# sergiventosa/ts-PWS

Measured on AMD Instinct MI355X. Metric: stacked samples/s (Morlet ts-PWS, 10k×131072) + % HBM roofline, 1/2/4/8 GPU, higher is better.
Workload: dtype f64; 1 GPU; 10000 traces/GPU x 131072 samples, Morlet w0=pi*sqrt(2/ln2) V=4 J=14, two-stage K=10 + unbiased phase coherence (BASELINE configs[2]); HBM-resident float32 traces; traces_total=10000, traces_per_gpu=10000, parallelism=one GPU: no collective, world_size=1

## Files before the change

### include/tspws_hip.h

```cpp
#ifndef TSPWS_HIP_H
#define TSPWS_HIP_H

#include <stddef.h>
#include <stdint.h>
#include "ts_pws1f_lib.h"

#ifdef __cplusplus
extern "C" {
#endif

enum {
	TSPWS_OK        = 0,
	TSPWS_E_ARG     = -1,
	TSPWS_E_NOMEM   = 4,
	TSPWS_E_NODEV   = 5,
	TSPWS_E_HIP     = 6,
	TSPWS_E_FRAME   = 7
};

typedef struct tspws_hip_plan tspws_hip_plan;

typedef struct {
	int      type;
	unsigned S, V, J, N;
	double   s0, b0, w0;
	double   Cpsi;
	size_t   ncoef;
	size_t   ntaps;
	int      device;
} tspws_hip_frame_info;

int         tspws_hip_device_count(void);
const char *tspws_hip_last_error(void);
int  tspws_hip_alloc(void **d_ptr, size_t bytes, int device);
int  tspws_hip_free(void *d_ptr);
int  tspws_hip_upload(void *d_dst, const void *h_src, size_t bytes, void *stream);
int  tspws_hip_download(void *h_dst, const void *d_src, size_t bytes, void *stream);
int  tspws_hip_zero(void *d_ptr, size_t bytes, void *stream);
int  tspws_hip_sync(void *stream);


void tspws_resolve_params(t_tsPWS *p, unsigned nsamp, float dt);

int  tspws_hip_plan_create(tspws_hip_plan **plan, int type, unsigned J, unsigned V, unsigned N,
                           double s0, double b0, double w0, int uni, int device);
void tspws_hip_plan_destroy(tspws_hip_plan *plan);
int  tspws_hip_plan_info(const tspws_hip_plan *plan, tspws_hip_frame_info *info);
int  tspws_hip_plan_tables(const tspws_hip_plan *plan, double *scale, unsigned *L, int *c, int *cd,
                           unsigned *D, unsigned *Ns);
int  tspws_hip_plan_taps(const tspws_hip_plan *plan, double *h_w, double *h_wd);

int  tspws_hip_fold(float *d_sigall, size_t mtr, size_t max, size_t ld, void *stream);
int  tspws_hip_remove_mean(float *d_sigall, size_t mtr, size_t max, size_t ld, void *stream);

int  tspws_hip_partial_stacks(tspws_hip_plan *plan, const float *d_sigall, size_t ld,
                              size_t mtr_local, size_t first, size_t mtr_global, unsigned Kmax,
                              double *d_P, size_t ldP, void *stream);

int  tspws_hip_partial_stacks_range(tspws_hip_plan *plan, const float *d_sigall, size_t ld,
                                    size_t mtr_local, size_t first, size_t mtr_global, unsigned Kmax,
                                    unsigned g_begin, unsigned g_end, double *d_P, size_t ldP, void *stream);

int  tspws_hip_forward_f64(tspws_hip_plan *plan, const double *d_x, size_t ntr, size_t ld, double *d_Y, void *stream);
int  tspws_hip_forward_f32(tspws_hip_plan *plan, const float  *d_x, size_t ntr, size_t ld, double *d_Y, void *stream);
unsigned tspws_hip_spectral_first_scale(const tspws_hip_plan *plan, unsigned nsmax);
unsigned tspws_hip_spectral_end_scale(const tspws_hip_plan *plan);
unsigned tspws_hip_spectral_transform_length(const tspws_hip_plan *plan);
unsigned tspws_hip_spectral_choice(const tspws_hip_plan *plan, size_t ntr);
int  tspws_hip_forward_spectral_f64(tspws_hip_plan *plan, const double *d_x, size_t ntr, size_t ld, double *d_Y, unsigned nsmax, void *stream);
int  tspws_hip_forward_spectral_f32(tspws_hip_plan *plan, const float  *d_x, size_t ntr, size_t ld, double *d_Y, unsigned nsmax, void *stream);
int  tspws_hip_inverse(tspws_hip_plan *plan, const double *d_Y, size_t nrec, double *d_x, void *stream);
typedef struct {
	unsigned items;
	unsigned per_scale;
	unsigned waves;
	unsigned waves_lds;
	unsigned waves_fast;
	unsigned generic;
} tspws_hip_inverse_info_t;
int  tspws_hip_inverse_info(const tspws_hip_plan *plan, tspws_hip_inverse_info_t *info);

int  tspws_hip_accumulate(tspws_hip_plan *plan, const double *d_Y, size_t ntr, double *d_ST, double *d_PS,
                          int zero_first, void *stream);
int  tspws_hip_stacks_double(tspws_hip_plan *plan, const double *d_P, unsigned K, size_t ldP,
                             double *d_ST, double *d_PS, void *stream);
int  tspws_hip_stacks_float(tspws_hip_plan *plan, const float *d_sigall, size_t mtr, size_t ld,
                            double *d_ST, double *d_PS, void *stream);
int  tspws_hip_weight(tspws_hip_plan *plan, double *d_OUT, const double *d_ST, const double *d_PS,
                      unsigned K, unsigned M, double wu, int unbiased, void *stream);
int  tspws_hip_epilogue(float *d_ls, float *d_tsPWS, const double *d_x_st, const double *d_x_out,
                        size_t N, unsigned mtr, void *stream);

int  tspws_hip_stack_local(tspws_hip_plan *plan, const t_tsPWS *p, const float *d_sigall, size_t ld,
                           size_t mtr_local, size_t first, size_t mtr_global, void *stream);
int  tspws_hip_reduce_buffer(tspws_hip_plan *plan, const t_tsPWS *p, size_t mtr_global,
                             double **d_buf, size_t *ndoubles);
int  tspws_hip_stack_finish(tspws_hip_plan *plan, const t_tsPWS *p, size_t mtr_global,
                            float *d_ls, float *d_tsPWS, void *stream);

int  tspws_hip_stack_finish_range(tspws_hip_plan *plan, const t_tsPWS *p, size_t mtr_global,
                                  unsigned g_begin, unsigned g_end, void *stream);
int  tspws_hip_stack_finish_tail(tspws_hip_plan *plan, const t_tsPWS *p, size_t mtr_global,
                                 float *d_ls, float *d_tsPWS, void *stream);

int  tspws_hip_stack(tspws_hip_plan *plan, const t_tsPWS *p, const float *d_sigall, size_t ld, size_t mtr,
                     float *d_ls, float *d_tsPWS, void *stream);
int  tspws_hip_stack_batch(tspws_hip_plan *plan, const t_tsPWS *p, const float *d_sigall, size_t ld, const size_t *h_first, unsigned B,
                           float *d_ls, float *d_tsPWS, void *stream);
typedef struct {
	unsigned single_pass;
	unsigned two_stage_pass;
	unsigned looped;
	unsigned empty;
	unsigned rounds;
// ... 187 lines not shown
```

### ts-pws_amd/__init__.py

```python
import ctypes as C
import os
import subprocess

_HERE = os.path.dirname(os.path.abspath(__file__))
ROOT = os.path.dirname(_HERE)
LIB_PATH = os.environ.get("TSPWS_LIB_PATH") or os.path.join(_HERE, "lib", "libtspws_hip.so")

time_t = C.c_long


class t_tsPWS(C.Structure):
    _fields_ = [
        ("type", C.c_int), ("uni", C.c_uint), ("J", C.c_uint), ("V", C.c_uint),
        ("s0", C.c_double), ("b0", C.c_double), ("w0", C.c_double), ("wu", C.c_double),
        ("fmin", C.c_double), ("Q", C.c_double), ("cycle", C.c_double),
        ("w0set", C.c_int), ("lrm", C.c_int), ("bin", C.c_int), ("lkinst", C.c_int),
        ("lVfix", C.c_int), ("ls0fix", C.c_int), ("lb0fix", C.c_int), ("verbose", C.c_int),
        ("fold", C.c_int), ("unbiased", C.c_int), ("convergence", C.c_int),
        ("subsmpl_N", C.c_uint), ("subsmpl_p", C.c_double),
        ("jackknife_n", C.c_uint), ("jackknife_d", C.c_uint), ("obin", C.c_uint),
        ("AllSteps", C.c_int), ("Nmax", C.c_uint), ("Kmax", C.c_uint),
        ("kinst", C.c_char_p), ("filein", C.c_char_p), ("fileout", C.c_char_p), ("fileconv", C.c_char_p),
    ]


class FrameInfo(C.Structure):
    _fields_ = [
        ("type", C.c_int), ("S", C.c_uint), ("V", C.c_uint), ("J", C.c_uint), ("N", C.c_uint),
        ("s0", C.c_double), ("b0", C.c_double), ("w0", C.c_double), ("Cpsi", C.c_double),
        ("ncoef", C.c_size_t), ("ntaps", C.c_size_t), ("device", C.c_int),
    ]


class InverseInfo(C.Structure):
    _fields_ = [("items", C.c_uint), ("per_scale", C.c_uint), ("waves", C.c_uint), ("waves_lds", C.c_uint), ("waves_fast", C.c_uint),
                ("generic", C.c_uint)]


class TspwsError(RuntimeError):
    pass


def build(verbose=False):
    out = subprocess.run(["make", "-C", _HERE, "all"], capture_output=True, text=True)
    if verbose or out.returncode:
        print(out.stdout + out.stderr)
    if out.returncode:
        raise TspwsError("building libtspws_hip.so failed")
    return LIB_PATH


_lib = None

_vp, _u, _d, _sz, _i, _f = C.c_void_p, C.c_uint, C.c_double, C.c_size_t, C.c_int, C.c_float
SYMBOLS = {
    "tspws_main": (_i, [_vp, _vp, _vp]),
    "tspws_hip_device_count": (_i, []),
    "tspws_hip_last_error": (C.c_char_p, []),
    "tspws_hip_alloc": (_i, [C.POINTER(_vp), _sz, _i]),
    "tspws_hip_free": (_i, [_vp]),
    "tspws_hip_upload": (_i, [_vp, _vp, _sz, _vp]),
    "tspws_hip_download": (_i, [_vp, _vp, _sz, _vp]),
    "tspws_hip_zero": (_i, [_vp, _sz, _vp]),
    "tspws_hip_sync": (_i, [_vp]),
    "tspws_resolve_params": (None, [_vp, _u, _f]),
    "tspws_hip_plan_create": (_i, [C.POINTER(_vp), _i, _u, _u, _u, _d, _d, _d, _i, _i]),
    "tspws_hip_plan_destroy": (None, [_vp]),
    "tspws_hip_plan_info": (_i, [_vp, _vp]),
    "tspws_hip_plan_tables": (_i, [_vp] + [_vp] * 6),
    "tspws_hip_plan_taps": (_i, [_vp, _vp, _vp]),
    "tspws_hip_fold": (_i, [_vp, _sz, _sz, _sz, _vp]),
    "tspws_hip_remove_mean": (_i, [_vp, _sz, _sz, _sz, _vp]),
    "tspws_hip_partial_stacks": (_i, [_vp, _vp, _sz, _sz, _sz, _sz, _u, _vp, _sz, _vp]),
    "tspws_hip_partial_stacks_range": (_i, [_vp, _vp, _sz, _sz, _sz, _sz, _u, _u, _u, _vp, _sz, _vp]),
    "tspws_hip_forward_f64": (_i, [_vp, _vp, _sz, _sz, _vp, _vp]),
    "tspws_hip_forward_f32": (_i, [_vp, _vp, _sz, _sz, _vp, _vp]),
    "tspws_hip_spectral_first_scale": (_u, [_vp, _u]),
    "tspws_hip_spectral_end_scale": (_u, [_vp]),
    "tspws_hip_spectral_transform_length": (_u, [_vp]),
    "tspws_hip_spectral_choice": (_u, [_vp, _sz]),
    "tspws_hip_forward_spectral_f64": (_i, [_vp, _vp, _sz, _sz, _vp, _u, _vp]),
    "tspws_hip_forward_spectral_f32": (_i, [_vp, _vp, _sz, _sz, _vp, _u, _vp]),
    "tspws_hip_inverse": (_i, [_vp, _vp, _sz, _vp, _vp]),
    "tspws_hip_inverse_info": (_i, [_vp, _vp]),
    "tspws_hip_accumulate": (_i, [_vp, _vp, _sz, _vp, _vp, _i, _vp]),
    "tspws_hip_stacks_double": (_i, [_vp, _vp, _u, _sz, _vp, _vp, _vp]),
    "tspws_hip_stacks_float": (_i, [_vp, _vp, _sz, _sz, _vp, _vp, _vp]),
    "tspws_hip_weight": (_i, [_vp, _vp, _vp, _vp, _u, _u, _d, _i, _vp]),
    "tspws_hip_epilogue": (_i, [_vp, _vp, _vp, _vp, _sz, _u, _vp]),
    "tspws_hip_stack_local": (_i, [_vp, _vp, _vp, _sz, _sz, _sz, _sz, _vp]),
    "tspws_hip_reduce_buffer": (_i, [_vp, _vp, _sz, C.POINTER(_vp), C.POINTER(_sz)]),
    "tspws_hip_stack_finish": (_i, [_vp, _vp, _sz, _vp, _vp, _vp]),
    "tspws_hip_stack_finish_range": (_i, [_vp, _vp, _sz, _u, _u, _vp]),
    "tspws_hip_stack_finish_tail": (_i, [_vp, _vp, _sz, _vp, _vp, _vp]),
    "tspws_hip_stack": (_i, [_vp, _vp, _vp, _sz, _sz, _vp, _vp, _vp]),
    "tspws_hip_stack_batch": (_i, [_vp, _vp, _vp, _sz, _vp, _u, _vp, _vp, _vp]),
    "tspws_hip_stack_batch_stats": (_i, [_vp, _vp]),
    "tspws_hip_profile_begin": (_i, [_vp, _sz]),
    "tspws_hip_profile_read": (_i, [_vp, _vp, _vp, _sz, C.POINTER(_sz)]),
    "tspws_hip_profile_end": (_i, [_vp, C.POINTER(_d), C.POINTER(_sz)]),
    "tspws_hip_stream_launches": (_i, [_vp]),
    "tspws_jackknife_plan": (_i, [_vp, _vp, _sz, _u, _u, _u]),
    "tspws_hip_jackknife": (_i, [_vp, _vp, _vp, _sz, _sz, _vp, _u, _vp, _vp, _vp, _vp]),
    "tspws_hip_stack_jackknife": (_i, [_vp, _vp, _vp, _sz, _sz, _vp, _vp, _vp, _u, _vp, _vp, _vp, _vp]),
    "tspws_main_release": (None, []),
    "tspws_main_on": (_i, [_i, _vp, _vp, _vp]),
    "tspws_main_cached_devices": (C.c_ulonglong, []),
    "tspws_hip_finish_shard": (_i, [_vp, _vp, _sz, _u, _u, C.POINTER(_u), C.POINTER(_u)]),
    "tspws_hip_stack_finish_scales": (_i, [_vp, _vp, _sz, _u, _u, _vp, _vp]),
    "tspws_hip_jackknife_buffer": (_i, [_vp, _vp, _u, C.POINTER(_vp), C.POINTER(_sz)]),
    "tspws_hip_jackknife_local": (_i, [_vp, _vp, _vp, _sz, _sz, _sz, _sz, _vp, _u, _vp]),
    "tspws_hip_jackknife_finish": (_i, [_vp, _vp, _sz, _vp, _u, _u, _u, _vp, _vp, _vp, _vp]),
    "tspws_selection_classes": (_i, [_vp, _u, _sz, _vp, _vp, C.POINTER(_u)]),
    "tspws_hip_jackknife_single": (_i, [_vp, _vp, _vp, _sz, _sz, _vp, _u, _vp, _vp, _vp, _vp]),
    "tspws_hip_jackknife_batch": (_i, [_vp, _vp, _vp, _sz, _vp, _u, _vp, _u, _vp, _vp, _vp, _vp, _vp, _vp]),
    "tspws_hip_jackknife_batch_stats": (_i, [_vp, _vp]),
    "tspws_hip_jackknife_batch_two_stage": (_i, [_vp, _vp, _vp, _sz, _vp, _u, _vp, _u, _vp, _vp, _vp, _vp, _vp, _vp]),
    "tspws_hip_jackknife_batch_two_stage_stats": (_i, [_vp, _vp]),
    "tspws_subsampling_plan": (_i, [_vp, _sz, _sz]),
    "tspws_hip_subsample": (_i, [_vp, _vp, _vp, _sz, _sz, _u, _vp, _vp, _vp]),
    "tspws_hip_subsample_sel": (_i, [_vp, _vp, _vp, _sz, _sz, _u, _vp, _vp, _vp, _vp]),
    "tspws_subsampling_plan_batch": (_i, [_vp, _vp, _u, _u, _d]),
    "tspws_hip_subsample_batch_sel": (_i, [_vp, _vp, _vp, _sz, _vp, _u, _u, _vp, _vp, _vp, _vp, _vp]),
    "tspws_hip_subsample_batch": (_i, [_vp, _vp, _vp, _sz, _vp, _u, _u, _vp, _vp, _vp, _vp]),
    "tspws_hip_subsample_batch_stats": (_i, [_vp, _vp]),
    "tspws_bootstrap_plan": (_i, [_vp, _sz]),
    "tspws_bootstrap_plan_batch": (_i, [_vp, _vp, _u, _u]),
    "tspws_hip_bootstrap_batch_cnt": (_i, [_vp, _vp, _vp, _sz, _vp, _u, _u, _vp, _vp, _vp, _vp, _vp, _vp]),
    "tspws_hip_bootstrap_batch": (_i, [_vp, _vp, _vp, _sz, _vp, _u, _u, _vp, _vp, _vp, _vp, _vp]),
    "tspws_hip_bootstrap_batch_stats": (_i, [_vp, _vp]),
    "tspws_hip_weighted_stack_batch": (_i, [_vp, _vp, _vp, _sz, _vp, _u, _u, _vp, _vp, _vp, _vp, _vp, _vp]),
    "tspws_hip_weighted_stack_batch_stats": (_i, [_vp, _vp]),
    "tspws_weights_from_scores": (_i, [_vp, _vp, _vp, _u, _i, _d]),
    "tspws_hip_replica_bands": (_i, [_vp, _vp, _sz, _u, _u, _vp, _vp, _u, _vp, _vp]),
    "tspws_hip_replica_bands_stats": (_i, [_vp, _vp]),
    "tspws_hip_trace_scores": (_i, [_vp, _vp, _sz, _vp, _u, _vp, _sz, _u, _sz, _sz, _vp, _vp, _vp]),
    "tspws_hip_trace_scores_stats": (_i, [_vp, _vp]),
    "tspws_selection_from_scores": (_i, [_vp, _vp, _vp, _vp, _u, _i, _d]),
    "tspws_hip_selective_stack_batch": (_i, [_vp, _vp, _vp, _sz, _vp, _u, _i, _i, _d, _u, _sz, _sz, _vp, _vp, _vp, _vp, _vp, _vp]),
    "tspws_hip_convergence": (_i, [_vp, _vp, _vp, _sz, _sz, _vp, _vp, _vp, _vp, _vp, _vp, _vp, _vp, _vp]),
    "tspws_hip_convergence_batch": (_i, [_vp, _vp, _vp, _sz, _vp, _u, _vp, _vp, _vp, _vp, _vp, _vp, _vp, _vp, _vp]),
    "tspws_hip_convergence_batch_stats": (_i, [_vp, _vp]),
    "tspws_hip_synth": (_i, [_vp, _sz, _sz, _sz, C.c_uint64, _sz, _vp]),
    "tspws_hip_comm_create": (_i, [C.POINTER(_vp), _i, _vp]),
    "tspws_hip_comm_destroy": (None, [_vp]),
    "tspws_hip_comm_size": (_i, [_vp]),
    "tspws_hip_comm_device": (_i, [_vp, _i]),
    "tspws_hip_comm_stream": (_vp, [_vp, _i]),
    "tspws_hip_comm_backend": (C.c_char_p, [_vp]),
    "tspws_hip_allreduce_f64": (_i, [_vp, _vp, _sz, _vp]),
    "tspws_hip_reduce_f64": (_i, [_vp, _vp, _sz, _i, _vp]),
    "tspws_shard_range": (None, [_sz, _u, _u, C.POINTER(_sz), C.POINTER(_sz)]),
    "tspws_hip_multi_create": (_i, [C.POINTER(_vp), _i, _vp, _i, _u, _u, _u, _d, _d, _d, _i]),
    "tspws_hip_multi_destroy": (None, [_vp]),
    "tspws_hip_multi_comm": (_vp, [_vp]),
    "tspws_hip_multi_plan": (_vp, [_vp, _i]),
    "tspws_hip_multi_upload": (_i, [_vp, _vp, _sz, _sz, C.POINTER(_vp), C.POINTER(_vp), C.POINTER(_vp)]),
    "tspws_hip_multi_prologue": (_i, [_vp, _vp, _sz, _sz, _sz, _i, _i]),
    "tspws_hip_multi_stack": (_i, [_vp, _vp, _vp, _sz, _sz, _vp, _vp]),
    "tspws_hip_multi_stack_jackknife": (_i, [_vp, _vp, _vp, _sz, _sz, _vp, _vp, _vp, _u, _vp, _vp, _vp]),
}


def load():
    global _lib
    if _lib is None:
        if not os.path.exists(LIB_PATH):
            raise TspwsError(f"{LIB_PATH} is missing: run __graft_entry__.build() / make -C ts-pws_amd")
        try:
            import torch
        except ImportError:
            pass
        lib = C.CDLL(LIB_PATH)
        for name, (res, args) in SYMBOLS.items():
            fn = getattr(lib, name)
            fn.restype, fn.argtypes = res, args
        _lib = lib
    return _lib


def check(rc, what=""):
    if rc:
        raise TspwsError(f"{what} failed with code {rc}: {load().tspws_hip_last_error().decode()}")


def resolve(params, nsamp, dt=1.0):
    p = t_tsPWS.from_buffer_copy(params)
    load().tspws_resolve_params(C.byref(p), nsamp, dt)
    return p


def shard_range(mtr_global, rank, world):
    first = rank * mtr_global // world
    last = (rank + 1) * mtr_global // world
    return first, last - first


class Plan:

    def __init__(self, params, N, device=0):
        self.lib = load()
        self.params = t_tsPWS.from_buffer_copy(params)
        h = C.c_void_p()
        p = self.params
        check(self.lib.tspws_hip_plan_create(C.byref(h), p.type, p.J, p.V, N, p.s0, p.b0, p.w0, int(p.uni), device), "plan_create")
        self.h = h
        info = FrameInfo()
        check(self.lib.tspws_hip_plan_info(self.h, C.byref(info)), "plan_info")
        self.info = info
        self.N, self.S, self.ncoef, self.ntaps, self.Cpsi = N, info.S, info.ncoef, info.ntaps, info.Cpsi
        self.device = device

    def tables(self):
        import numpy as np
        S = self.S
        t = dict(scale=np.zeros(S), L=np.zeros(S, np.uint32), c=np.zeros(S, np.int32), cd=np.zeros(S, np.int32),
# ... 41 lines not shown
        return t.data_ptr()

    def stacks(self, traces):
        import numpy as np
        import torch
        if traces.dtype not in (torch.float32, torch.float64):
            raise TspwsError(f"traces must be float32 or float64 [mtr][{self.N}], got {traces.dtype}")
        mtr, ld = self._traces(traces, traces.dtype)
        if not mtr:
            raise TspwsError("stacks needs at least one row")
        fn = self.lib.tspws_hip_stacks_float if traces.dtype == torch.float32 else self.lib.tspws_hip_stacks_double
        ST = torch.full((2 * self.ncoef,), float("nan"), dtype=torch.float64, device=traces.device)
        PS = torch.full((2 * self.ncoef,), float("nan"), dtype=torch.float64, device=traces.device)
        check(fn(self.h, traces.data_ptr(), mtr, ld, ST.data_ptr(), PS.data_ptr(), self._stream()), "stacks")
        torch.cuda.synchronize(traces.device)
        return ST.cpu().numpy().view(np.complex128), PS.cpu().numpy().view(np.complex128)

    def inverse_info(self):
        info = InverseInfo()
        check(self.lib.tspws_hip_inverse_info(self.h, C.byref(info)), "inverse_info")
        return {k: int(getattr(info, k)) for k, _ in InverseInfo._fields_}

    def inverse(self, Y):
        import numpy as np
        import torch
        if isinstance(Y, np.ndarray):
            if Y.dtype != np.complex128 or Y.ndim != 2 or Y.shape[1] != self.ncoef or not Y.shape[0]:
                raise TspwsError(f"Y must be complex128 [nrec >= 1][{self.ncoef}], got {Y.dtype} {Y.shape}")
            Yd = torch.as_tensor(np.ascontiguousarray(Y), device=f"cuda:{self.device}")
        elif isinstance(Y, torch.Tensor):
            if Y.dtype != torch.complex128 or Y.dim() != 2 or Y.shape[1] != self.ncoef or not Y.shape[0]:
                raise TspwsError(f"Y must be complex128 [nrec >= 1][{self.ncoef}], got {Y.dtype} {tuple(Y.shape)}")
            if not Y.is_cuda or (Y.device.index or 0) != self.device or not Y.is_contiguous():
                raise TspwsError(f"Y must be a contiguous tensor on cuda:{self.device}, got {Y.device}")
            Yd = Y
        else:
            raise TspwsError("Y must be a complex128 numpy array or device tensor")
        x = torch.full((Yd.shape[0], self.N), float("nan"), dtype=torch.float64, device=Yd.device)
        check(self.lib.tspws_hip_inverse(self.h, Yd.data_ptr(), Yd.shape[0], x.data_ptr(), self._stream()), "inverse")
        torch.cuda.synchronize(Yd.device)
        return x.cpu().numpy() if isinstance(Y, np.ndarray) else x

    def stack_local(self, traces, first=0, mtr_global=None):
        mtr, ld = self._traces(traces)
        mtr_global = mtr if mtr_global is None else mtr_global
        check(self.lib.tspws_hip_stack_local(self.h, C.byref(self.params), traces.data_ptr(), ld, mtr, first, mtr_global, self._stream()),
              "stack_local")

    def partial_stacks_range(self, traces, first, mtr_global, g_begin, g_end):
        mtr, ld = self._traces(traces)
        buf = self.reduce_buffer(mtr_global)
        check(self.lib.tspws_hip_partial_stacks_range(self.h, traces.data_ptr(), ld, mtr, first, mtr_global, self.params.Kmax, g_begin, g_end,
                                                      buf.data_ptr(), self.N, self._stream()), "partial_stacks_range")

    def stack_finish(self, mtr_global, ls, ts):
        check(self.lib.tspws_hip_stack_finish(self.h, C.byref(self.params), mtr_global, self._out(ls, "ls"), self._out(ts, "ts"), self._stream()),
              "stack_finish")

    def stack_finish_range(self, mtr_global, g_begin, g_end):
        check(self.lib.tspws_hip_stack_finish_range(self.h, C.byref(self.params), mtr_global, g_begin, g_end, self._stream()),
              "stack_finish_range")

    def stack_finish_tail(self, mtr_global, ls, ts):
        check(self.lib.tspws_hip_stack_finish_tail(self.h, C.byref(self.params), mtr_global, self._out(ls, "ls"), self._out(ts, "ts"),
                                                   self._stream()), "stack_finish_tail")

    @staticmethod
    def _sel(sel, C_, mtr_global):
        import numpy as np
        sel = np.ascontiguousarray(sel, dtype=np.int8)
        if sel.shape != (C_, mtr_global):
            raise TspwsError(f"selection must be [{C_}][{mtr_global}] (replica x trace of the WHOLE ensemble), got {sel.shape}")
        return sel

    def jackknife_buffer(self, C_):
        import torch
        ptr, n = C.c_void_p(), C.c_size_t()
        check(self.lib.tspws_hip_jackknife_buffer(self.h, C.byref(self.params), C_, C.byref(ptr), C.byref(n)), "jackknife_buffer")
        return _as_tensor(ptr.value, n.value, torch.float64, self.device)

    def jackknife_local(self, traces, first, mtr_global, sel):
        mtr, ld = self._traces(traces)
        sel = self._sel(sel, sel.shape[0], mtr_global)
        check(self.lib.tspws_hip_jackknife_local(self.h, C.byref(self.params), traces.data_ptr(), ld, mtr, first, mtr_global, sel.ctypes.data,
                                                 sel.shape[0], self._stream()), "jackknife_local")

    def jackknife_finish(self, mtr_global, sel, c_begin, c_end, ls_out, ts_out, mtr_out):
        import torch
        import numpy as np
        sel = self._sel(sel, sel.shape[0], mtr_global)
        if not isinstance(mtr_out, np.ndarray) or mtr_out.dtype != np.uint32 or mtr_out.shape != (sel.shape[0],) or not mtr_out.flags.c_contiguous:
            raise TspwsError(f"mtr_out must be a contiguous uint32 numpy array of {sel.shape[0]} entries")
        for t, name in ((ls_out, "ls_out"), (ts_out, "ts_out")):
            if t.dtype != torch.float32 or tuple(t.shape) != (sel.shape[0], self.N) or not t.is_contiguous() or not t.is_cuda or \
                    (t.device.index or 0) != self.device:
                raise TspwsError(f"{name} must be a contiguous float32 [{sel.shape[0]}][{self.N}] tensor on cuda:{self.device}")
        check(self.lib.tspws_hip_jackknife_finish(self.h, C.byref(self.params), mtr_global, sel.ctypes.data, sel.shape[0], c_begin, c_end,
                                                  ls_out.data_ptr(), ts_out.data_ptr(), mtr_out.ctypes.data, self._stream()), "jackknife_finish")

    def finish_shard(self, mtr_global, rank, world):
        a, b = C.c_uint(), C.c_uint()
        rc = self.lib.tspws_hip_finish_shard(self.h, C.byref(self.params), mtr_global, rank, world, C.byref(a), C.byref(b))
        if rc == 1:
            return None
        check(rc, "finish_shard")
        return a.value, b.value
# ... 729 lines not shown
```

### ts-pws_amd/csrc/stream.hip

```cpp
#include "tspws_internal.h"
#include <hip/hip_ext.h>

__global__ void __launch_bounds__(256) k_fold(float *__restrict__ x, size_t max, size_t ld)
{
	float *row = x + (size_t)blockIdx.y * ld;
	const size_t half = max / 2;
	for (size_t n = (size_t)blockIdx.x * blockDim.x + threadIdx.x; n < half; n += (size_t)gridDim.x * blockDim.x) {
		float v = row[n];
		v += row[max - 1 - n];
		v *= 0.5f;
		row[max - 1 - n] = v;
		row[n] = v;
	}
}

__global__ void __launch_bounds__(1024) k_remove_mean(float *__restrict__ x, size_t max, size_t ld)
{
	__shared__ double part[16];
	__shared__ float meanf;
	float *row = x + (size_t)blockIdx.x * ld;
	double acc = 0;
	for (size_t n = threadIdx.x; n < max; n += blockDim.x) acc += (double)row[n];
	acc = wave_sum(acc);
	if ((threadIdx.x & 63) == 0) part[threadIdx.x >> 6] = acc;
// ... 433 lines not shown
	if (cached && p->ck_dev) {
		if (st != p->ck_stream) HIP_TRY(hipStreamWaitEvent(st, p->ck_ev, 0));
		return 0;
	}
	p->ck_dev = false;
	if (nck) HIP_TRY(hipMemcpyAsync(*d_chunks, chunks.data(), nck * sizeof(Chunk), hipMemcpyHostToDevice, st));
	HIP_TRY(hipMemcpyAsync(*d_rf, row_first.data(), (rows + 1) * sizeof(unsigned), hipMemcpyHostToDevice, st));
	if (cached) {
		if ((rc = tspws_plan_event(p->ck_ev, true))) return rc;
		HIP_TRY(hipEventRecord(p->ck_ev, st));
		p->ck_stream = st;
		p->ck_dev = true;
	}
	return 0;
}

int tspws_run_chunks(tspws_hip_plan *p, const float *d_x, size_t ld, size_t N, const std::vector<Chunk> &chunks,
                     const std::vector<unsigned> &row_first, unsigned rows, double *d_P, size_t ldP, hipStream_t st, bool cached,
                     unsigned row_begin, unsigned row_end)
{
	int rc;
	if ((rc = tspws_chunks_upload(p, chunks, row_first, rows, st, cached))) return rc;
	return tspws_chunks_launch(p, d_x, ld, N, chunks, row_first, rows, d_P, ldP, st, row_begin, row_end);
}

int tspws_chunks_upload(tspws_hip_plan *p, const std::vector<Chunk> &chunks, const std::vector<unsigned> &row_first, unsigned rows, hipStream_t st,
                        bool cached)
{
	Chunk *d_chunks = nullptr;
	unsigned *d_rf = nullptr;
	p->jk_gen = 0;
	return chunk_tables(p, chunks, row_first, rows, st, cached, &d_chunks, &d_rf);
}

int tspws_chunks_launch(tspws_hip_plan *p, const float *d_x, size_t ld, size_t N, const std::vector<Chunk> &chunks,
                        const std::vector<unsigned> &row_first, unsigned rows, double *d_P, size_t ldP, hipStream_t st,
                        unsigned row_begin, unsigned row_end)
{
	row_end = std::min(row_end, rows);
	const size_t nck = chunks.size();
	const size_t ldpc = (N + 3) & ~(size_t)3;
	void *d_pc = nullptr;
	int rc;
	if ((rc = scratch(p, SCR_CHUNK, std::max<size_t>(nck * ldpc * sizeof(double), 16), &d_pc))) return rc;
	if (!p->scr[SCR_TAB]) return fail(TSPWS_E_ARG, "chunks_launch: no table uploaded");
	Chunk *d_chunks = (Chunk *)p->scr[SCR_TAB];
	unsigned *d_rf = (unsigned *)((char *)p->scr[SCR_TAB] + nck * sizeof(Chunk));
	if (row_begin >= row_end) return 0;
	const unsigned bx = (unsigned)((N + 1023) / 1024);
	const bool vec = (N % 4 == 0) && (ld % 4 == 0) && (((uintptr_t)d_x & 15) == 0);
	const size_t ck0 = row_first[row_begin], ck1 = row_first[row_end];
	bool direct = ck1 - ck0 == (size_t)(row_end - row_begin) && ck1 - ck0 <= 65535 && (!vec || ldP % 2 == 0);
	for (unsigned r = row_begin; r < row_end && direct; r++) direct = row_first[r + 1] - row_first[r] == 1;
	if (direct) {
		const unsigned wg_target = 256;
		size_t rows_total = 0;
		for (size_t c = ck0; c < ck1; c++) rows_total += chunks[c].count;
		const bool long_runs = ck1 > ck0 && rows_total / (ck1 - ck0) >= 256;
		const unsigned rpl = long_runs ? std::max(1u, wg_target / std::max(1u, bx)) : 65535u;
		p->last_stream_launches = 0;
		for (size_t c0 = ck0; c0 < ck1; c0 += rpl) {
			p->last_stream_launches++;
			const unsigned ny = (unsigned)std::min<size_t>(ck1 - c0, rpl);
			double *dst = d_P + (size_t)(row_begin + (c0 - ck0)) * ldP;
			hipEvent_t e0 = nullptr, e1 = nullptr;
			if (c0 == ck0) { e0 = p->le.first_start; p->le.first_start = nullptr; }
			if (c0 + rpl >= ck1) { e1 = p->le.last_stop; p->le.last_stop = nullptr; p->le.ready = e1; }
			if (e0 || e1) {
				if (vec) hipExtLaunchKernelGGL(k_partial<true>, dim3(bx, ny), dim3(256), 0, st, e0, e1, 0, d_x, ld, N, (const Chunk *)(d_chunks + c0), dst, ldP);
				else hipExtLaunchKernelGGL(k_partial<false>, dim3(bx, ny), dim3(256), 0, st, e0, e1, 0, d_x, ld, N, (const Chunk *)(d_chunks + c0), dst, ldP);
			} else if (vec) hipLaunchKernelGGL(k_partial<true>, dim3(bx, ny), dim3(256), 0, st, d_x, ld, N, d_chunks + c0, dst, ldP);
			else hipLaunchKernelGGL(k_partial<false>, dim3(bx, ny), dim3(256), 0, st, d_x, ld, N, d_chunks + c0, dst, ldP);
		}
		HIP_TRY(hipGetLastError());
		return 0;
	}
	p->last_stream_launches = 0;
	for (size_t c0 = ck0; c0 < ck1; c0 += 65535) {
		p->last_stream_launches++;
		const unsigned ny = (unsigned)std::min<size_t>(ck1 - c0, 65535);
		hipEvent_t e0 = nullptr;
		if (c0 == ck0) { e0 = p->le.first_start; p->le.first_start = nullptr; }
		if (e0) {
			if (vec) hipExtLaunchKernelGGL(k_partial<true>, dim3(bx, ny), dim3(256), 0, st, e0, nullptr, 0, d_x, ld, N, (const Chunk *)(d_chunks + c0), (double *)d_pc + c0 * ldpc, ldpc);
			else hipExtLaunchKernelGGL(k_partial<false>, dim3(bx, ny), dim3(256), 0, st, e0, nullptr, 0, d_x, ld, N, (const Chunk *)(d_chunks + c0), (double *)d_pc + c0 * ldpc, ldpc);
		} else if (vec) hipLaunchKernelGGL(k_partial<true>, dim3(bx, ny), dim3(256), 0, st, d_x, ld, N, d_chunks + c0, (double *)d_pc + c0 * ldpc, ldpc);
		else hipLaunchKernelGGL(k_partial<false>, dim3(bx, ny), dim3(256), 0, st, d_x, ld, N, d_chunks + c0, (double *)d_pc + c0 * ldpc, ldpc);
	}
	for (unsigned r0 = row_begin; r0 < row_end; r0 += 65535) {
		const unsigned ny = std::min(row_end - r0, 65535u);
		hipEvent_t e1 = nullptr;
		if (r0 + 65535u >= row_end) { e1 = p->le.last_stop; p->le.last_stop = nullptr; p->le.ready = e1; }
		if (e1) hipExtLaunchKernelGGL(k_reduce_chunks, dim3((unsigned)((N + 255) / 256), ny), dim3(256), 0, st, nullptr, e1, 0, (const double *)d_pc, ldpc,
		                              (const unsigned *)(d_rf + r0), d_P + (size_t)r0 * ldP, ldP, N);
		else hipLaunchKernelGGL(k_reduce_chunks, dim3((unsigned)((N + 255) / 256), ny), dim3(256), 0, st, (const double *)d_pc, ldpc,
		                        d_rf + r0, d_P + (size_t)r0 * ldP, ldP, N);
	}
	HIP_TRY(hipGetLastError());
	return 0;
}

unsigned tspws_chunk_len_for(size_t N, size_t mtr)
{
	const size_t colblocks = (N + 1023) / 1024;
	const size_t want = std::max<size_t>(1, 1024 / std::max<size_t>(colblocks, 1));
	size_t len = (mtr + want - 1) / want;
	len = std::max<size_t>(len, 8);
	return (unsigned)std::min<size_t>(len, 1u << 20);
}

static void build_group_chunks(tspws_hip_plan *p, size_t mtr_local, size_t first, size_t mtr_global, unsigned Kmax)
{
	if (p->ck_valid && p->ck_mtr == mtr_local && p->ck_first == first && p->ck_glob == mtr_global && p->ck_K == Kmax) return;
	p->ck_dev = false;
	p->chunks.clear();
	p->row_first.assign(Kmax + 1, 0);
	const unsigned clen = tspws_chunk_len_for(p->N, mtr_local);
	std::vector<std::vector<Chunk>> per(Kmax);
	size_t i = 0;
	while (i < mtr_local) {
		const size_t g = (size_t)floor((double)((first + i) * (size_t)Kmax) / (double)mtr_global);
		size_t j = i + 1;
		while (j < mtr_local && (size_t)floor((double)((first + j) * (size_t)Kmax) / (double)mtr_global) == g) j++;
		const size_t n = j - i, pieces = (n + clen - 1) / clen, base = n / pieces, rem = n % pieces;
		size_t t = i;
		for (size_t k = 0; k < pieces; k++) {
			Chunk c; c.t0 = t; c.count = (unsigned)(base + (k < rem ? 1 : 0)); c.row = (unsigned)g;
			per[std::min<size_t>(g, Kmax - 1)].push_back(c);
			t += c.count;
		}
		i = j;
	}
	for (unsigned g = 0; g < Kmax; g++) {
		p->row_first[g] = (unsigned)p->chunks.size();
		p->chunks.insert(p->chunks.end(), per[g].begin(), per[g].end());
	}
	p->row_first[Kmax] = (unsigned)p->chunks.size();
	p->ck_mtr = mtr_local; p->ck_first = first; p->ck_glob = mtr_global; p->ck_K = Kmax; p->ck_valid = true;
}

extern "C" int tspws_hip_partial_stacks(tspws_hip_plan *p, const float *d_x, size_t ld, size_t mtr_local, size_t first,
                                        size_t mtr_global, unsigned Kmax, double *d_P, size_t ldP, void *stream)
{
	if (!p || (!d_x && mtr_local) || !d_P || !Kmax || !mtr_global || first + mtr_local > mtr_global)
		return fail(TSPWS_E_ARG, "partial_stacks: bad argument");
	HIP_TRY(hipSetDevice(p->device));
	build_group_chunks(p, mtr_local, first, mtr_global, Kmax);
	return tspws_run_chunks(p, d_x, ld, p->N, p->chunks, p->row_first, Kmax, d_P, ldP, S_(stream), true);
}

extern "C" int tspws_hip_partial_stacks_range(tspws_hip_plan *p, const float *d_x, size_t ld, size_t mtr_local, size_t first,
                                              size_t mtr_global, unsigned Kmax, unsigned g_begin, unsigned g_end, double *d_P, size_t ldP,
                                              void *stream)
{
	if (!p || (!d_x && mtr_local) || !d_P || !Kmax || !mtr_global || g_begin > g_end || g_end > Kmax || first + mtr_local > mtr_global)
		return fail(TSPWS_E_ARG, "partial_stacks_range: bad argument");
	HIP_TRY(hipSetDevice(p->device));
	build_group_chunks(p, mtr_local, first, mtr_global, Kmax);
	return tspws_run_chunks(p, d_x, ld, p->N, p->chunks, p->row_first, Kmax, d_P, ldP, S_(stream), true, g_begin, g_end);
}
```

### ts-pws_amd/csrc/tspws_internal.h

```cpp
#pragma once

#include <hip/hip_runtime.h>

#include <algorithm>
#include <cmath>
#include <cstdio>
#include <cstdlib>
#include <cstring>
#include <string>
#include <vector>

#include "tspws_hip.h"

#ifndef TSPWS_PI
#define TSPWS_PI 3.14159265358979328
#endif

int tspws_fail(int code, const char *what, hipError_t e = hipSuccess);
#define fail tspws_fail

#define HIP_TRY(expr)                                                              \
	do {                                                                           \
		hipError_t e_ = (expr);                                                    \
		if (e_ != hipSuccess) return tspws_fail(e_ == hipErrorOutOfMemory ? TSPWS_E_NOMEM : TSPWS_E_HIP, #expr, e_); \
// ... 272 lines not shown
int  tspws_stacks(tspws_hip_plan *p, const TIn *d_x, size_t ntr, size_t ld, double *d_ST, double *d_PS, hipStream_t st, bool keep,
                  const WeightArgs *wa, bool *weighted, ScaleRange rg);
unsigned tspws_first_unfused_scale(const tspws_hip_plan *p);
void tspws_launch_accumulate(tspws_hip_plan *p, const double2 *part, unsigned nb, double2 *ST, double2 *PS, int zero_first, const FuseOut *fz,
                             unsigned nslices, hipStream_t st, unsigned nbatch, size_t y_part, size_t y_stack, const TlTable *tl, const WeightArgs *wa,
                             ScaleRange rg, const AccExtra *ex = nullptr);
bool tspws_fused_forward(const tspws_hip_plan *p);
bool tspws_many_trace_path(const tspws_hip_plan *p, size_t ntr);
unsigned tspws_spectral_choice(const tspws_hip_plan *p, size_t ntr);
size_t tspws_part_budget_bytes();
int  tspws_engine_pin();
bool tspws_generic_forward();
unsigned tspws_spectral_first_scale(const tspws_hip_plan *p, unsigned nsmax);
int  tspws_spectral_decomp(tspws_hip_plan *p, unsigned s_first, unsigned nblk_hint, SpecDecomp **out, bool few = false);
int  tspws_spectral_rows_f64(tspws_hip_plan *p, SpecDecomp *dc, const double *d_x, size_t ld, unsigned ntr, unsigned tps, const FuseOut &fz, hipStream_t st,
                             hipEvent_t after_transposition = nullptr);
int  tspws_build_tl_spectral(tspws_hip_plan *p, unsigned s_first, unsigned s_end, unsigned nblk_hint, TlTable &T);
void tspws_spectral_geometry(const tspws_hip_plan *p, unsigned *NT, unsigned *s_end, unsigned *cneg);
unsigned tspws_spectral_end_scale(const tspws_hip_plan *p);
struct SpecRowsOut;
template <typename TIn>
int  tspws_spectral_run(tspws_hip_plan *p, SpecDecomp *dc, const TIn *xT, unsigned TP, unsigned ntr, double2 *ST, double2 *PS, size_t stride, double2 *Y, hipStream_t st,
                        const SpecRowsOut *ro = nullptr, unsigned tps = 0, unsigned ncol = 0);
template <typename TIn>
int  tspws_spectral_transpose(tspws_hip_plan *p, const TIn *d_x, size_t ld, unsigned ntr, TIn *xT, unsigned TP, hipStream_t st);
void tspws_spectral_destroy(tspws_hip_plan *p);
int  tspws_build_inverse(tspws_hip_plan *p);
size_t tspws_inverse_row_bytes(const tspws_hip_plan *p);
int  tspws_weight_mode(double wu, int unbiased, unsigned K);
void tspws_weight_batched(tspws_hip_plan *p, double2 *OUT, const double2 *ST, const double2 *PS, int mode, double K, double wu, const double *d_Mv,
                          unsigned nb, size_t y_out, size_t y_stack, hipStream_t st, double M = 0.0);
int  tspws_inverse_pair_out(tspws_hip_plan *p, const double2 *Y, float *d_ts, float *d_ls, float mtr, hipStream_t st);
int  tspws_inverse_scales(tspws_hip_plan *p, const double2 *Y, double *x2, hipStream_t st, ScaleRange rg);
int  tspws_inverse_pairs_early(tspws_hip_plan *p, const double2 *Y, unsigned nb, unsigned s_split, hipStream_t early, bool *done);
int  tspws_inverse_pairs_late(tspws_hip_plan *p, const double2 *Y, double *x, unsigned nb, unsigned s_split, hipStream_t st);
bool tspws_generic_inverse();
void tspws_epilogue_rows(float *d_ts, const double *d_x, size_t N, unsigned nb, hipStream_t st);
int  tspws_run_chunks(tspws_hip_plan *p, const float *d_x, size_t ld, size_t N, const std::vector<Chunk> &chunks,
                      const std::vector<unsigned> &row_first, unsigned rows, double *d_P, size_t ldP, hipStream_t st, bool cached,
                      unsigned row_begin = 0, unsigned row_end = ~0u);
int  tspws_chunks_upload(tspws_hip_plan *p, const std::vector<Chunk> &chunks, const std::vector<unsigned> &row_first, unsigned rows, hipStream_t st,
                         bool cached);
int  tspws_chunks_launch(tspws_hip_plan *p, const float *d_x, size_t ld, size_t N, const std::vector<Chunk> &chunks,
                         const std::vector<unsigned> &row_first, unsigned rows, double *d_P, size_t ldP, hipStream_t st,
                         unsigned row_begin = 0, unsigned row_end = ~0u);
int  tspws_prefix_launch(tspws_hip_plan *p, const float *d_x, size_t ld, size_t N, const Chunk *d_runs, const unsigned *d_seg_first, unsigned nseg,
                         size_t nruns_total, const unsigned *d_carry, unsigned ncarry, double **d_snap, size_t *ldpc, hipStream_t st);
void tspws_combine_terms_launch(const double *d_snap, size_t ldpc, const unsigned *d_row_ptr, const unsigned *d_idx, const float *d_coef, unsigned nrows,
                                double *d_P, size_t N, hipStream_t st);
int  tspws_rows_walk_launch(const float *d_x, size_t ld, size_t N, const RunDesc *d_runs, unsigned q0, unsigned qm, unsigned q1, unsigned W,
                            const unsigned *d_flush_rows, const unsigned *d_fix_row, double *d_rows, double *d_blk, int carry_in, int carry_out, hipStream_t st);
unsigned tspws_rows_walk_wmax();
unsigned tspws_chunk_len_for(size_t N, size_t mtr);
class BatchCall;
int  tspws_jb2_shared(tspws_hip_plan *p, const t_tsPWS *par, const float *d_x, size_t ld, const size_t *h_first, const unsigned *list, size_t n,
                      const char *h_sel, size_t Tn, unsigned C, bool main, float *d_ls, float *d_ts, float *d_ls_out, float *d_ts_out, unsigned *h_mtr_out,
                      BatchCall &call, tspws_hip_jk_batch2_stats *stats);
bool tspws_is_two_stage(const t_tsPWS *p, size_t mtr_global);
```

Before: 1356 billion samples/s.

## Balance trace pieces across partial-stack launches via makespan-aware chunk splitting

Chunk construction for partial stacks moves into a planner that models each launch's makespan as the longest piece in it. When runs are long, it searches piece totals near the default, in steps of the pieces-per-launch count, and keeps a split that evens piece lengths and reduces launch count with a per-launch overhead term. The non-direct path now also batches launches by the same pieces-per-launch rule rather than a fixed 65535. It adds host-side planning cost and an env override, and exposes the plan to Python for inspection.

```diff
diff --git a/include/tspws_hip.h b/include/tspws_hip.h
--- a/include/tspws_hip.h
+++ b/include/tspws_hip.h
@@ -60,6 +60,12 @@
 int  tspws_hip_partial_stacks_range(tspws_hip_plan *plan, const float *d_sigall, size_t ld,
                                     size_t mtr_local, size_t first, size_t mtr_global, unsigned Kmax,
                                     unsigned g_begin, unsigned g_end, double *d_P, size_t ldP, void *stream);
+
+typedef struct { unsigned long long t0; unsigned count; unsigned row; } tspws_stream_piece;
+int  tspws_stream_plan(size_t N, size_t mtr_local, size_t first, size_t mtr_global, unsigned Kmax,
+                       tspws_stream_piece *pieces, size_t cap_pieces, size_t *npieces,
+                       unsigned *launch_first, size_t cap_launches, size_t *nlaunches,
+                       size_t *makespan, size_t *makespan_legacy);
 
 int  tspws_hip_forward_f64(tspws_hip_plan *plan, const double *d_x, size_t ntr, size_t ld, double *d_Y, void *stream);
 int  tspws_hip_forward_f32(tspws_hip_plan *plan, const float  *d_x, size_t ntr, size_t ld, double *d_Y, void *stream);
diff --git a/ts-pws_amd/__init__.py b/ts-pws_amd/__init__.py
--- a/ts-pws_amd/__init__.py
+++ b/ts-pws_amd/__init__.py
@@ -73,6 +73,7 @@
     "tspws_hip_remove_mean": (_i, [_vp, _sz, _sz, _sz, _vp]),
     "tspws_hip_partial_stacks": (_i, [_vp, _vp, _sz, _sz, _sz, _sz, _u, _vp, _sz, _vp]),
     "tspws_hip_partial_stacks_range": (_i, [_vp, _vp, _sz, _sz, _sz, _sz, _u, _u, _u, _vp, _sz, _vp]),
+    "tspws_stream_plan": (_i, [_sz, _sz, _sz, _sz, _u, _vp, _sz, C.POINTER(_sz), _vp, _sz, C.POINTER(_sz), C.POINTER(_sz), C.POINTER(_sz)]),
     "tspws_hip_forward_f64": (_i, [_vp, _vp, _sz, _sz, _vp, _vp]),
     "tspws_hip_forward_f32": (_i, [_vp, _vp, _sz, _sz, _vp, _vp]),
     "tspws_hip_spectral_first_scale": (_u, [_vp, _u]),
@@ -162,6 +163,20 @@
 }
 
 
+def stream_plan(N, mtr_local, first, mtr_global, Kmax):
+    import numpy as np
+    lib = load()
+    npc, nl, span, legacy = _sz(), _sz(), _sz(), _sz()
+    args = (N, mtr_local, first, mtr_global, Kmax)
+    if lib.tspws_stream_plan(*args, None, 0, C.byref(npc), None, 0, C.byref(nl), C.byref(span), C.byref(legacy)):
+        raise TspwsError(f"stream_plan: bad argument {args}")
+    pieces = np.zeros(max(1, npc.value), dtype=np.dtype([("t0", "<u8"), ("count", "<u4"), ("row", "<u4")]))
+    lf = np.zeros(nl.value + 1, dtype=np.uint32)
+    lib.tspws_stream_plan(*args, pieces.ctypes.data, npc.value, None, lf.ctypes.data, nl.value, None, None, None)
+    return {"pieces": [(int(t0), int(c), int(r)) for t0, c, r in pieces[:npc.value]], "launch_first": [int(v) for v in lf],
+            "makespan": span.value, "makespan_legacy": legacy.value}
+
+
 def load():
     global _lib
     if _lib is None:
@@ -309,6 +324,9 @@
         buf = self.reduce_buffer(mtr_global)
         check(self.lib.tspws_hip_partial_stacks_range(self.h, traces.data_ptr(), ld, mtr, first, mtr_global, self.params.Kmax, g_begin, g_end,
                                                       buf.data_ptr(), self.N, self._stream()), "partial_stacks_range")
+
+    def stream_plan(self, mtr_local, first=0, mtr_global=None):
+        return stream_plan(self.N, mtr_local, first, mtr_local if mtr_global is None else mtr_global, self.params.Kmax)
 
     def stack_finish(self, mtr_global, ls, ts):
         check(self.lib.tspws_hip_stack_finish(self.h, C.byref(self.params), mtr_global, self._out(ls, "ls"), self._out(ts, "ts"), self._stream()),
diff --git a/ts-pws_amd/csrc/stream.hip b/ts-pws_amd/csrc/stream.hip
--- a/ts-pws_amd/csrc/stream.hip
+++ b/ts-pws_amd/csrc/stream.hip
@@ -509,40 +509,26 @@
 	const size_t ck0 = row_first[row_begin], ck1 = row_first[row_end];
 	bool direct = ck1 - ck0 == (size_t)(row_end - row_begin) && ck1 - ck0 <= 65535 && (!vec || ldP % 2 == 0);
 	for (unsigned r = row_begin; r < row_end && direct; r++) direct = row_first[r + 1] - row_first[r] == 1;
+	const size_t rpl = tspws_pieces_per_launch(N, chunks, ck0, ck1);
+	double *const out = direct ? d_P + (size_t)row_begin * ldP : (double *)d_pc + ck0 * ldpc;
+	const size_t ldo = direct ? ldP : ldpc;
+	p->last_stream_launches = 0;
+	for (size_t c0 = ck0; c0 < ck1; c0 += rpl) {
+		p->last_stream_launches++;
+		const unsigned ny = (unsigned)std::min<size_t>(ck1 - c0, rpl);
+		double *dst = out + (c0 - ck0) * ldo;
+		hipEvent_t e0 = nullptr, e1 = nullptr;
+		if (c0 == ck0) { e0 = p->le.first_start; p->le.first_start = nullptr; }
+		if (direct && c0 + rpl >= ck1) { e1 = p->le.last_stop; p->le.last_stop = nullptr; p->le.ready = e1; }
+		if (e0 || e1) {
+			if (vec) hipExtLaunchKernelGGL(k_partial<true>, dim3(bx, ny), dim3(256), 0, st, e0, e1, 0, d_x, ld, N, (const Chunk *)(d_chunks + c0), dst, ldo);
+			else hipExtLaunchKernelGGL(k_partial<false>, dim3(bx, ny), dim3(256), 0, st, e0, e1, 0, d_x, ld, N, (const Chunk *)(d_chunks + c0), dst, ldo);
+		} else if (vec) hipLaunchKernelGGL(k_partial<true>, dim3(bx, ny), dim3(256), 0, st, d_x, ld, N, d_chunks + c0, dst, ldo);
+		else hipLaunchKernelGGL(k_partial<false>, dim3(bx, ny), dim3(256), 0, st, d_x, ld, N, d_chunks + c0, dst, ldo);
+	}
 	if (direct) {
-		const unsigned wg_target = 256;
-		size_t rows_total = 0;
-		for (size_t c = ck0; c < ck1; c++) rows_total += chunks[c].count;
-		const bool long_runs = ck1 > ck0 && rows_total / (ck1 - ck0) >= 256;
-		const unsigned rpl = long_runs ? std::max(1u, wg_target / std::max(1u, bx)) : 65535u;
-		p->last_stream_launches = 0;
-		for (size_t c0 = ck0; c0 < ck1; c0 += rpl) {
-			p->last_stream_launches++;
-			const unsigned ny = (unsigned)std::min<size_t>(ck1 - c0, rpl);
-			double *dst = d_P + (size_t)(row_begin + (c0 - ck0)) * ldP;
-			hipEvent_t e0 = nullptr, e1 = nullptr;
-			if (c0 == ck0) { e0 = p->le.first_start; p->le.first_start = nullptr; }
-			if (c0 + rpl >= ck1) { e1 = p->le.last_stop; p->le.last_stop = nullptr; p->le.ready = e1; }
-			if (e0 || e1) {
-				if (vec) hipExtLaunchKernelGGL(k_partial<true>, dim3(bx, ny), dim3(256), 0, st, e0, e1, 0, d_x, ld, N, (const Chunk *)(d_chunks + c0), dst, ldP);
-				else hipExtLaunchKernelGGL(k_partial<false>, dim3(bx, ny), dim3(256), 0, st, e0, e1, 0, d_x, ld, N, (const Chunk *)(d_chunks + c0), dst, ldP);
-			} else if (vec) hipLaunchKernelGGL(k_partial<true>, dim3(bx, ny), dim3(256), 0, st, d_x, ld, N, d_chunks + c0, dst, ldP);
-			else hipLaunchKernelGGL(k_partial<false>, dim3(bx, ny), dim3(256), 0, st, d_x, ld, N, d_chunks + c0, dst, ldP);
-		}
 		HIP_TRY(hipGetLastError());
 		return 0;
-	}
-	p->last_stream_launches = 0;
-	for (size_t c0 = ck0; c0 < ck1; c0 += 65535) {
-		p->last_stream_launches++;
-		const unsigned ny = (unsigned)std::min<size_t>(ck1 - c0, 65535);
-		hipEvent_t e0 = nullptr;
-		if (c0 == ck0) { e0 = p->le.first_start; p->le.first_start = nullptr; }
-		if (e0) {
-			if (vec) hipExtLaunchKernelGGL(k_partial<true>, dim3(bx, ny), dim3(256), 0, st, e0, nullptr, 0, d_x, ld, N, (const Chunk *)(d_chunks + c0), (double *)d_pc + c0 * ldpc, ldpc);
-			else hipExtLaunchKernelGGL(k_partial<false>, dim3(bx, ny), dim3(256), 0, st, e0, nullptr, 0, d_x, ld, N, (const Chunk *)(d_chunks + c0), (double *)d_pc + c0 * ldpc, ldpc);
-		} else if (vec) hipLaunchKernelGGL(k_partial<true>, dim3(bx, ny), dim3(256), 0, st, d_x, ld, N, d_chunks + c0, (double *)d_pc + c0 * ldpc, ldpc);
-		else hipLaunchKernelGGL(k_partial<false>, dim3(bx, ny), dim3(256), 0, st, d_x, ld, N, d_chunks + c0, (double *)d_pc + c0 * ldpc, ldpc);
 	}
 	for (unsigned r0 = row_begin; r0 < row_end; r0 += 65535) {
 		const unsigned ny = std::min(row_end - r0, 65535u);
@@ -557,42 +543,11 @@
 	return 0;
 }
 
-unsigned tspws_chunk_len_for(size_t N, size_t mtr)
-{
-	const size_t colblocks = (N + 1023) / 1024;
-	const size_t want = std::max<size_t>(1, 1024 / std::max<size_t>(colblocks, 1));
-	size_t len = (mtr + want - 1) / want;
-	len = std::max<size_t>(len, 8);
-	return (unsigned)std::min<size_t>(len, 1u << 20);
-}
-
 static void build_group_chunks(tspws_hip_plan *p, size_t mtr_local, size_t first, size_t mtr_global, unsigned Kmax)
 {
 	if (p->ck_valid && p->ck_mtr == mtr_local && p->ck_first == first && p->ck_glob == mtr_global && p->ck_K == Kmax) return;
 	p->ck_dev = false;
-	p->chunks.clear();
-	p->row_first.assign(Kmax + 1, 0);
-	const unsigned clen = tspws_chunk_len_for(p->N, mtr_local);
-	std::vector<std::vector<Chunk>> per(Kmax);
-	size_t i = 0;
-	while (i < mtr_local) {
-		const size_t g = (size_t)floor((double)((first + i) * (size_t)Kmax) / (double)mtr_global);
-		size_t j = i + 1;
-		while (j < mtr_local && (size_t)floor((double)((first + j) * (size_t)Kmax) / (double)mtr_global) == g) j++;
-		const size_t n = j - i, pieces = (n + clen - 1) / clen, base = n / pieces, rem = n % pieces;
-		size_t t = i;
-		for (size_t k = 0; k < pieces; k++) {
-			Chunk c; c.t0 = t; c.count = (unsigned)(base + (k < rem ? 1 : 0)); c.row = (unsigned)g;
-			per[std::min<size_t>(g, Kmax - 1)].push_back(c);
-			t += c.count;
-		}
-		i = j;
-	}
-	for (unsigned g = 0; g < Kmax; g++) {
-		p->row_first[g] = (unsigned)p->chunks.size();
-		p->chunks.insert(p->chunks.end(), per[g].begin(), per[g].end());
-	}
-	p->row_first[Kmax] = (unsigned)p->chunks.size();
+	tspws_group_chunks(p->N, mtr_local, first, mtr_global, Kmax, p->chunks, p->row_first, nullptr, nullptr);
 	p->ck_mtr = mtr_local; p->ck_first = first; p->ck_glob = mtr_global; p->ck_K = Kmax; p->ck_valid = true;
 }
 
diff --git a/ts-pws_amd/csrc/stream_plan.hip b/ts-pws_amd/csrc/stream_plan.hip
--- /dev/null
+++ b/ts-pws_amd/csrc/stream_plan.hip
@@ -0,0 +1,145 @@
+#include "tspws_internal.h"
+
+#include <algorithm>
+#include <cmath>
+#include <cstdlib>
+#include <vector>
+
+unsigned tspws_pieces_per_launch(size_t N, const std::vector<Chunk> &chunks, size_t ck0, size_t ck1)
+{
+	const unsigned wg_target = 256;
+	const unsigned bx = (unsigned)((N + 1023) / 1024);
+	size_t rows_total = 0;
+	for (size_t c = ck0; c < ck1; c++) rows_total += chunks[c].count;
+	const bool long_runs = ck1 > ck0 && rows_total / (ck1 - ck0) >= 256;
+	return long_runs ? std::max(1u, wg_target / std::max(1u, bx)) : 65535u;
+}
+
+unsigned tspws_chunk_len_for(size_t N, size_t mtr)
+{
+	const size_t colblocks = (N + 1023) / 1024;
+	const size_t want = std::max<size_t>(1, 1024 / std::max<size_t>(colblocks, 1));
+	size_t len = (mtr + want - 1) / want;
+	len = std::max<size_t>(len, 8);
+	return (unsigned)std::min<size_t>(len, 1u << 20);
+}
+
+namespace {
+
+struct Run { size_t t0, n; unsigned row; };
+
+inline size_t piece_len(size_t n, size_t p, size_t k) { return n / p + (k < n % p ? 1 : 0); }
+
+size_t makespan_of(const std::vector<Run> &runs, const std::vector<size_t> &pc, unsigned rpl, size_t *launches)
+{
+	size_t span = 0, in_launch = 0, longest = 0, nl = 0;
+	for (size_t g = 0; g < runs.size(); g++)
+		for (size_t k = 0; k < pc[g]; k++) {
+			longest = std::max(longest, piece_len(runs[g].n, pc[g], k));
+			if (++in_launch == rpl) { span += longest; nl++; in_launch = 0; longest = 0; }
+		}
+	if (in_launch) { span += longest; nl++; }
+	if (launches) *launches = nl;
+	return span;
+}
+
+bool split_total(const std::vector<Run> &runs, size_t mtr, size_t total, std::vector<size_t> &pc)
+{
+	const size_t G = runs.size();
+	if (total < G || total > mtr) return false;
+	pc.assign(G, 1);
+	std::vector<std::pair<double, size_t>> rem(G);
+	size_t sum = 0;
+	for (size_t g = 0; g < G; g++) {
+		const double q = (double)runs[g].n * (double)total / (double)mtr;
+		pc[g] = std::min(runs[g].n, std::max<size_t>(1, (size_t)floor(q)));
+		rem[g] = { q - (double)pc[g], g };
+		sum += pc[g];
+	}
+	std::stable_sort(rem.begin(), rem.end(), [](const std::pair<double, size_t> &a, const std::pair<double, size_t> &b) { return a.first > b.first; });
+	for (size_t pass = 0; sum < total && pass < total; pass++)
+		for (size_t k = 0; k < G && sum < total; k++)
+			if (pc[rem[k].second] < runs[rem[k].second].n) { pc[rem[k].second]++; sum++; }
+	for (size_t pass = 0; sum > total && pass < total; pass++)
+		for (size_t k = G; k-- > 0 && sum > total;)
+			if (pc[rem[k].second] > 1) { pc[rem[k].second]--; sum--; }
+	return sum == total;
+}
+
+}
+
+void tspws_group_chunks(size_t N, size_t mtr_local, size_t first, size_t mtr_global, unsigned Kmax, std::vector<Chunk> &chunks,
+                        std::vector<unsigned> &row_first, size_t *makespan, size_t *makespan_legacy)
+{
+	const size_t BOUNDARY = 16;
+	chunks.clear();
+	row_first.assign(Kmax + 1, 0);
+	std::vector<Run> runs;
+	for (size_t i = 0; i < mtr_local;) {
+		const size_t g = (size_t)floor((double)((first + i) * (size_t)Kmax) / (double)mtr_global);
+		size_t j = i + 1;
+		while (j < mtr_local && (size_t)floor((double)((first + j) * (size_t)Kmax) / (double)mtr_global) == g) j++;
+		runs.push_back({ i, j - i, (unsigned)g });
+		i = j;
+	}
+	size_t clen = tspws_chunk_len_for(N, mtr_local);
+	std::vector<size_t> pc(runs.size()), cand;
+	size_t total = 0;
+	bool several = false;
+	for (size_t g = 0; g < runs.size(); g++) {
+		pc[g] = (runs[g].n + clen - 1) / clen;
+		total += pc[g];
+		several = several || pc[g] > 1;
+	}
+	const unsigned bx = (unsigned)((N + 1023) / 1024);
+	const bool long_runs = total && mtr_local / total >= 256;
+	const unsigned rpl = long_runs ? std::max(1u, 256u / std::max(1u, bx)) : 65535u;
+	size_t launches = 0;
+	const size_t span_legacy = makespan_of(runs, pc, rpl, &launches);
+	size_t span = span_legacy;
+	if (long_runs && several) {
+		size_t target = clen;
+		if (const char *e = sweep_env("TSPWS_STREAM_PIECE")) target = (size_t)std::max(0, atoi(e));
+		size_t best = span_legacy + BOUNDARY * launches;
+		const size_t mid = std::max<size_t>(1, (mtr_local / std::max<size_t>(target, 1) + rpl / 2) / rpl) * rpl;
+		for (size_t t = mid > rpl ? mid - rpl : mid; target && t <= mid + rpl; t += rpl) {
+			if (mtr_local / t < 256 || !split_total(runs, mtr_local, t, cand)) continue;
+			const size_t s = makespan_of(runs, cand, rpl, &launches);
+			if (s <= span_legacy && s + BOUNDARY * launches < best) { best = s + BOUNDARY * launches; span = s; pc = cand; }
+		}
+	}
+	for (size_t g = 0; g < runs.size(); g++) {
+		const unsigned row = std::min(runs[g].row, Kmax - 1);
+		size_t t = runs[g].t0;
+		for (size_t k = 0; k < pc[g]; k++) {
+			Chunk c; c.t0 = t; c.count = (unsigned)piece_len(runs[g].n, pc[g], k); c.row = runs[g].row;
+			chunks.push_back(c);
+			t += c.count;
+			row_first[row + 1] = (unsigned)chunks.size();
+		}
+	}
+	for (unsigned g = 0; g < Kmax; g++) row_first[g + 1] = std::max(row_first[g + 1], row_first[g]);
+	if (makespan) *makespan = span;
+	if (makespan_legacy) *makespan_legacy = span_legacy;
+}
+
+extern "C" int tspws_stream_plan(size_t N, size_t mtr_local, size_t first, size_t mtr_global, unsigned Kmax, tspws_stream_piece *pieces,
+                                 size_t cap_pieces, size_t *npieces, unsigned *launch_first, size_t cap_launches, size_t *nlaunches,
+                                 size_t *makespan, size_t *makespan_legacy)
+{
+	if (!N || !Kmax || !mtr_global || first + mtr_local > mtr_global) return 1;
+	std::vector<Chunk> chunks;
+	std::vector<unsigned> row_first;
+	tspws_group_chunks(N, mtr_local, first, mtr_global, Kmax, chunks, row_first, makespan, makespan_legacy);
+	for (size_t c = 0; c < chunks.size() && c < cap_pieces && pieces; c++) {
+		pieces[c].t0 = chunks[c].t0; pieces[c].count = chunks[c].count; pieces[c].row = chunks[c].row;
+	}
+	if (npieces) *npieces = chunks.size();
+	const size_t rpl = tspws_pieces_per_launch(N, chunks, 0, chunks.size());
+	size_t nl = 0;
+	for (size_t c0 = 0; c0 < chunks.size(); c0 += rpl, nl++)
+		if (launch_first && nl < cap_launches) launch_first[nl] = (unsigned)c0;
+	if (launch_first && nl <= cap_launches) launch_first[nl] = (unsigned)chunks.size();
+	if (nlaunches) *nlaunches = nl;
+	return 0;
+}
diff --git a/ts-pws_amd/csrc/tspws_internal.h b/ts-pws_amd/csrc/tspws_internal.h
--- a/ts-pws_amd/csrc/tspws_internal.h
+++ b/ts-pws_amd/csrc/tspws_internal.h
@@ -348,6 +348,9 @@
                             const unsigned *d_flush_rows, const unsigned *d_fix_row, double *d_rows, double *d_blk, int carry_in, int carry_out, hipStream_t st);
 unsigned tspws_rows_walk_wmax();
 unsigned tspws_chunk_len_for(size_t N, size_t mtr);
+unsigned tspws_pieces_per_launch(size_t N, const std::vector<Chunk> &chunks, size_t ck0, size_t ck1);
+void tspws_group_chunks(size_t N, size_t mtr_local, size_t first, size_t mtr_global, unsigned Kmax, std::vector<Chunk> &chunks,
+                        std::vector<unsigned> &row_first, size_t *makespan, size_t *makespan_legacy);
 class BatchCall;
 int  tspws_jb2_shared(tspws_hip_plan *p, const t_tsPWS *par, const float *d_x, size_t ld, const size_t *h_first, const unsigned *list, size_t n,
                       const char *h_sel, size_t Tn, unsigned C, bool main, float *d_ls, float *d_ts, float *d_ls_out, float *d_ts_out, unsigned *h_mtr_out,
```

New measurement: 1357 billion samples/s, median of 2. No clear change (+0.0%).
